# Fireflies-17/Speech-Inpainting

Measured on AMD Instinct MI355X. Metric: real-time factor (audio-sec/wall-sec) per GPU, 4 s clips @16 kHz, 200 ms mask, higher is better.
Workload: dtype encoder GEMMs and attention products: bf16 MFMA, fp32 accumulate (softmax, LayerNorm, head, arg-max in fp32); vocoder: fp16 MFMA (operands rounded to fp16, saturating), fp32 accumulate, activations stored as fp16; 1 GPU; BASELINE configs[1]: batch=32 x 4 s clips per GPU, 200 ms mask, HuBERT-base + HiFi-GAN V1; step = masked log-mel front-end -> encoder -> arg-max/splice -> vocoder on resident raw clips; global_batch=32, clip_samples=64000, mask_frames=10, parallelism=utterance-sharded x1

## Files before the change

speech_inpainting_amd/csrc/api.hip:

```cpp
#include <cmath>
#include <cstdarg>
#include <cstdio>
#include <cstdlib>
#include <cstring>
#include <map>
#include <sstream>
#include <string>
#include <vector>

#include "common.h"

namespace {

struct HostTensor {
    const float* data = nullptr;
    std::vector<long> shape;
    long numel() const { long n = 1; for (long d : shape) n *= d; return n; }
};

struct GemmW {
    size_t w = 0, w_lo = 0, bias = 0;
    int Cin = 0, N = 0, Npad = 0, ntaps = 0, groups = 1, math = 0;
    bool has_bias = false;
};

struct LayerW { GemmW qkv, out, ffn1, ffn2; size_t ln1_g, ln1_b, ln2_g, ln2_b; };
struct ConvW { GemmW g; size_t ln_g = 0, ln_b = 0; };
struct ResW { GemmW c1[SI_MAX_DIL], c2[SI_MAX_DIL]; };

struct Layout {
    size_t total = 0;
    size_t conv0_w, conv0_bias, conv0_g, conv0_b;
    std::vector<ConvW> convs;
    size_t fp_ln_g, fp_ln_b; GemmW proj;
    GemmW pos; size_t enc_ln_g, enc_ln_b;
    std::vector<LayerW> layers;
    size_t head_ln_g, head_ln_b; GemmW head;
    size_t cb_centered, cb_raw, cb_rnorm;
    GemmW pre; std::vector<GemmW> ups; std::vector<ResW> rbs;
    size_t post_w, post_b; int post_C = 0;
    int mel_ld = 0;
};

}

struct si_ctx {
    int device = 0;
    si_model_desc d{};
    char err[512] = {0};
    Layout lay;
    char* wdev = nullptr;
    bool weights_ready = false;
    bool weights_verified = false;
    std::map<std::string, long> dbg_size;
    std::map<std::string, std::pair<float*, long>> dbg_capture;
    struct ProfRec { int name; hipEvent_t a, b; double flops, bytes; };
    bool prof_on = false;
    std::string prof_filter;
    std::vector<std::string> prof_names;
    std::vector<ProfRec> prof_recs;
    std::vector<hipEvent_t> prof_pool;
    size_t prof_used = 0;
    int prof_open = -1;
    int num_cus = 0;
    std::map<const void*, size_t> dyn_lds;
    bool opt_voc_opready = true, opt_voc_res16 = true, opt_enc_opready = true, opt_att_bf16 = true, opt_enc_lingemm = true;
    bool opt_enc_posconv = true;
    int opt_ln_fuse = 1;
    int opt_voc_upsgemm = 1;
    int opt_ffn_pad = 64;
    int opt_gemmcu = 1;
    int opt_voc_chain = 1;
    int opt_voc_fuse = 1;
    char* fe_dev = nullptr;
    size_t fe_dft = 0, fe_hann = 0, fe_basis = 0, fe_lo = 0, fe_hi = 0;
    std::vector<int32_t> vl_host;
    static constexpr int VL_SLOTS = 4;
    int32_t* vl_pin[VL_SLOTS] = {nullptr, nullptr, nullptr, nullptr};
    size_t vl_pin_ints[VL_SLOTS] = {0, 0, 0, 0};
    hipEvent_t vl_ev[VL_SLOTS] = {nullptr, nullptr, nullptr, nullptr};
    int vl_next = 0;
    float* km_cnorm = nullptr;
    int km_cnorm_cap = 0;
};

static char g_create_err[512] = "";

int si_fail(si_ctx* ctx, int code, const char* fmt, ...) {
    char* dst = ctx ? ctx->err : g_create_err;
    va_list ap;
    va_start(ap, fmt);
    vsnprintf(dst, 512, fmt, ap);
    va_end(ap);
    return code;
}
int si_fail_hip(si_ctx* ctx, hipError_t e, const char* what, const char* file, int line) {
    return si_fail(ctx, SI_EHIP, "HIP error %d (%s) at %s:%d: %s", (int)e, hipGetErrorString(e), file, line, what);
}

struct TapSrc { const void* p; long n; int esize = 4; long cols = 0, ld = 0; };
static int si_tap(si_ctx* ctx, hipStream_t st, TapSrc s, const char* fmt, int a = 0, int b = 0, int c = 0) {
    if (ctx->dbg_capture.empty() && strchr(fmt, '%')) return SI_OK;
    char name[48];
    snprintf(name, sizeof(name), fmt, a, b, c);
    ctx->dbg_size[name] = s.n;
    auto it = ctx->dbg_capture.find(name);
    if (it == ctx->dbg_capture.end()) return SI_OK;
    const long m = s.n < it->second.second ? s.n : it->second.second;
    if (m <= 0) return SI_OK;
    if (s.ld > s.cols && s.cols > 0) {
        if (m / s.cols > 0)
            SI_HIP_CHECK(hipMemcpy2DAsync(it->second.first, (size_t)s.cols * s.esize, s.p, (size_t)s.ld * s.esize, (size_t)s.cols * s.esize,
                                          (size_t)(m / s.cols), hipMemcpyDeviceToDevice, st));
    } else {
        SI_HIP_CHECK(hipMemcpyAsync(it->second.first, s.p, (size_t)m * s.esize, hipMemcpyDeviceToDevice, st));
    }
    return SI_OK;
}

void si_prof_begin(si_ctx* ctx, const char* name, double flops, double bytes, hipStream_t st) {
    if (!ctx->prof_on || ctx->prof_used + 2 > ctx->prof_pool.size()) { ctx->prof_open = -1; return; }
    if (!ctx->prof_filter.empty() && ctx->prof_filter != name) { ctx->prof_open = -1; return; }
    int id = -1;
    for (size_t i = 0; i < ctx->prof_names.size(); ++i) if (ctx->prof_names[i] == name) { id = (int)i; break; }
    if (id < 0) { id = (int)ctx->prof_names.size(); ctx->prof_names.push_back(name); }
    si_ctx::ProfRec r{id, ctx->prof_pool[ctx->prof_used], ctx->prof_pool[ctx->prof_used + 1], flops, bytes};
    ctx->prof_used += 2;
    (void)hipEventRecord(r.a, st);
    ctx->prof_open = (int)ctx->prof_recs.size();
    ctx->prof_recs.push_back(r);
}
const char* si_prof_shape_name(const char* name, long M, int N, int K) {
    static const bool on = getenv("SI_PROF_SHAPES") && atoi(getenv("SI_PROF_SHAPES")) != 0;
    if (!on) return name;
    static thread_local char buf[48];
    snprintf(buf, sizeof(buf), "%s_%ldx%dx%d", name, M, N, K);
    return buf;
}
int si_ensure_dyn_lds(si_ctx* ctx, const void* kern, size_t bytes) {
    if (bytes <= 64 * 1024) return SI_OK;
    size_t& have = ctx->dyn_lds[kern];
    if (bytes > have) {
        SI_HIP_CHECK(hipFuncSetAttribute(kern, hipFuncAttributeMaxDynamicSharedMemorySize, (int)bytes));
        have = bytes;
    }
    return SI_OK;
}
int si_opt_gemmcu(const si_ctx* ctx) { return ctx->opt_gemmcu; }
int si_num_cus(si_ctx* ctx) {
    if (ctx->num_cus <= 0) {
        int n = 0;
        if (hipDeviceGetAttribute(&n, hipDeviceAttributeMultiprocessorCount, ctx->device) != hipSuccess || n <= 0) n = 256;
        ctx->num_cus = n;
    }
    return ctx->num_cus;
}
static int vl_upload(si_ctx* ctx, int32_t* dst, hipStream_t st) {
    const size_t n = ctx->vl_host.size();
    const int slot = ctx->vl_next;
    ctx->vl_next = (slot + 1) % si_ctx::VL_SLOTS;
    if (!ctx->vl_ev[slot]) SI_HIP_CHECK(hipEventCreateWithFlags(&ctx->vl_ev[slot], hipEventDisableTiming));
    else SI_HIP_CHECK(hipEventSynchronize(ctx->vl_ev[slot]));
    if (ctx->vl_pin_ints[slot] < n) {
        if (ctx->vl_pin[slot]) SI_HIP_CHECK(hipHostFree(ctx->vl_pin[slot]));
        ctx->vl_pin[slot] = nullptr; ctx->vl_pin_ints[slot] = 0;
        SI_HIP_CHECK(hipHostMalloc(reinterpret_cast<void**>(&ctx->vl_pin[slot]), std::max<size_t>(n, 4096) * sizeof(int32_t), hipHostMallocDefault));
        ctx->vl_pin_ints[slot] = std::max<size_t>(n, 4096);
    }
    memcpy(ctx->vl_pin[slot], ctx->vl_host.data(), n * sizeof(int32_t));
    SI_HIP_CHECK(hipMemcpyAsync(dst, ctx->vl_pin[slot], n * sizeof(int32_t), hipMemcpyHostToDevice, st));
    SI_HIP_CHECK(hipEventRecord(ctx->vl_ev[slot], st));
    return SI_OK;
}
void si_prof_end(si_ctx* ctx, hipStream_t st) {
    if (ctx->prof_open < 0) return;
    (void)hipEventRecord(ctx->prof_recs[ctx->prof_open].b, st);
    ctx->prof_open = -1;
}

namespace {

size_t elem_bytes(int math) { return math == SI_MATH_F32 ? 4 : 2; }

struct Planner {
    size_t cur = 0;
    size_t take(size_t bytes) { size_t o = cur; cur += (bytes + 255) / 256 * 256; return o; }
    size_t floats(size_t n) { return take(n * 4); }
    GemmW gemm(int math, int groups, int ntaps, int N, int Cin, bool bias) {
        GemmW g;
        g.math = math; g.groups = groups; g.ntaps = ntaps; g.N = N; g.Cin = Cin; g.has_bias = bias;
        g.Npad = si_round_up(N, si_pick_bn(N));
        const size_t n = (size_t)groups * ntaps * g.Npad * Cin;
        g.w = take(n * elem_bytes(math));
        if (math == SI_MATH_BF16X3) g.w_lo = take(n * 2);
        if (bias) g.bias = floats((size_t)groups * N);
        return g;
    }
};

int stage_channels(const si_ctx* ctx, int i) {
    const int real = ctx->d.up_initial_channel >> (i + 1);
    const bool r16 = ctx->opt_voc_opready && ctx->opt_voc_res16 && ctx->d.vocoder_math == SI_MATH_F16;
    return (r16 && real < 32 && real >= 4) ? 32 : real;
}

int plan_layout(si_ctx* ctx) {
    const si_model_desc& d = ctx->d;
    Layout& L = ctx->lay;
    Planner P;
    P.take(256);
    const int em = d.encoder_math, vm = d.vocoder_math;
    const int H = d.hidden_size;
    L.conv0_w = P.floats((size_t)d.conv_dim[0] * d.conv_kernel[0]);
    L.conv0_bias = d.conv_bias ? P.floats(d.conv_dim[0]) : 0;
    L.conv0_g = P.floats(d.conv_dim[0]);
    L.conv0_b = P.floats(d.conv_dim[0]);
    L.convs.clear();
    for (int i = 1; i < d.num_conv; ++i) {
        ConvW c;
        c.g = P.gemm(em, 1, d.conv_kernel[i], d.conv_dim[i], d.conv_dim[i - 1], d.conv_bias != 0);
        if (d.feat_norm_layer) { c.ln_g = P.floats(d.conv_dim[i]); c.ln_b = P.floats(d.conv_dim[i]); }
        L.convs.push_back(c);
    }
    const int CF = d.conv_dim[d.num_conv - 1];
    L.fp_ln_g = P.floats(CF); L.fp_ln_b = P.floats(CF);
    L.proj = P.gemm(em, 1, 1, H, CF, true);
    L.pos = P.gemm(em, d.pos_conv_groups, d.pos_conv_kernel, H / d.pos_conv_groups, H / d.pos_conv_groups, true);
    L.enc_ln_g = P.floats(H); L.enc_ln_b = P.floats(H);
    L.layers.clear();
    for (int l = 0; l < d.num_layers; ++l) {
        LayerW w;
// ... 346 lines not shown
    size_t f = 2 * (size_t)B * cmax + BT * d.conv_dim[d.num_conv - 1] + BT * d.hidden_size * 3 + BT * 3 * d.hidden_size + BT * d.intermediate_size +
               (size_t)B * d.conv_dim[0] * 2 + BT * 2;
    const size_t h16 = (BT * d.conv_dim[d.num_conv - 1] + 2 * BT * d.hidden_size + BT * (d.intermediate_size + 128)) * 2;
    return f * 4 + h16 + (size_t)B * 16 + (size_t)B * 4 + si_conv0_partials_bytes(B, N) + 41 * 256 +
           align_up((size_t)(SI_MAX_CONV + 3) * (B + 1) * 4, 256);
}

int vocoder_chunk(const si_model_desc& d, int B) { int c = d.vocoder_chunk > 0 ? d.vocoder_chunk : 32; return std::min(c, std::max(B, 1)); }

long voc_tout(int Tm, int stretch) { return stretch ? (long)std::floor((double)Tm * (441.0 / 256.0)) : Tm; }

size_t vocoder_ws_bytes(const si_ctx* ctx, int B, int Tm, int stretch) {
    const si_model_desc& d = ctx->d;
    const int Bc = vocoder_chunk(d, B);
    const long Tout = voc_tout(Tm, stretch);
    size_t lc_max = (size_t)Tout * d.up_initial_channel;
    long L = Tout; int c = d.up_initial_channel;
    for (int i = 0; i < d.num_ups; ++i) { L *= d.up_rates[i]; c = stage_channels(ctx, i); lc_max = std::max(lc_max, (size_t)L * c); }
    const size_t f = (size_t)Bc * Tout * ctx->lay.mel_ld + 9 * (size_t)Bc * lc_max;
    return f * 4 + 32 * 256 + align_up((size_t)(2 * SI_MAX_UPS + 3) * B * 4, 256);
}

TapGemmParams gemm_params(const si_ctx* ctx, const GemmW& G) {
    TapGemmParams p{};
    p.w = ctx->wdev + G.w;
    p.w_lo = G.math == SI_MATH_BF16X3 ? ctx->wdev + G.w_lo : nullptr;
    p.bias = G.has_bias ? reinterpret_cast<const float*>(ctx->wdev + G.bias) : nullptr;
    p.Cin = G.Cin; p.N = G.N; p.Npad = G.Npad; p.ntaps = G.ntaps; p.groups = G.groups;
    p.stride = 1; p.dil = 1; p.pad = 0; p.pro_slope = 1.f; p.act = SI_ACT_NONE; p.alpha = 1.f; p.accumulate = 0;
    p.out16_slope = 1.f;
    p.nseg = 1;
    return p;
}

struct UpsGeom { int u, pad; long Lout; int M; };
UpsGeom ups_geom(const si_model_desc& d, int i, long Lin) {
    const int u = d.up_rates[i], pad = (d.up_kernels[i] - u) / 2;
    const long Lout = Lin * u;
    return UpsGeom{u, pad, Lout, (int)((pad + Lout - 1) / u + 1)};
}

struct ResLn { const float* stats = nullptr; const float* gamma = nullptr; const float* beta = nullptr; };
struct LinearIo { const unsigned short* x16 = nullptr; unsigned short* y16 = nullptr; int ld_in = 0, ld_out = 0; ResLn res_ln; };
int linear(si_ctx* ctx, const GemmW& G, const float* x, float* y, long rows, int act, const float* res, hipStream_t st, const LinearIo& io = LinearIo()) {
    TapGemmParams p = gemm_params(ctx, G);
    p.x = io.x16 ? nullptr : x; p.x16 = io.x16; p.out = y; p.out16 = io.y16; p.res = res; p.act = act;
    p.res_stats = io.res_ln.stats; p.res_gamma = io.res_ln.gamma; p.res_beta = io.res_ln.beta;
    p.nseg = 1; p.Lin = (int)rows; p.M = (int)rows; p.ldx = io.ld_in ? io.ld_in : G.Cin; p.x_seg_stride = 0;
    p.ldo = io.ld_out ? io.ld_out : G.N; p.o_seg_stride = 0; p.ooff = 0; p.olimit = rows * p.ldo;
    p.lingemm = ctx->opt_enc_lingemm;
    return si_launch_tapgemm(ctx, G.math, p, st);
}

const float* wf(const si_ctx* ctx, size_t off) { return reinterpret_cast<const float*>(ctx->wdev + off); }

}

static int hubert_run(si_ctx* ctx, const float* wav, const int32_t* mask_start, const int32_t* mask_len, const int32_t* valid_len,
                      int normalize, float norm_eps, const double* pre_add, int output_layer, int B, int N, float* out_feats, float* out_hidden,
                      void* workspace, size_t workspace_bytes, si_stream_t stream, const int32_t* host_len = nullptr);

extern "C" {

int si_version(void) { return SI_ABI_VERSION; }

const char* si_last_error(const si_ctx* ctx) { return ctx ? ctx->err : g_create_err; }

int si_create(si_ctx** out, int device_id, const si_model_desc* desc) {
    if (!out) return si_fail(nullptr, SI_EINVAL, "si_create: out is NULL");
    *out = nullptr;
    int rc = check_desc(nullptr, desc);
    if (rc) return rc;
    int ndev = 0;
    if (hipGetDeviceCount(&ndev) != hipSuccess || device_id < 0 || device_id >= ndev)
        return si_fail(nullptr, SI_EHIP, "si_create: device %d not available (%d HIP devices visible)", device_id, ndev);
    si_ctx* ctx = new si_ctx();
    ctx->device = device_id;
    ctx->d = *desc;
    auto env_flag = [](const char* name) { const char* v = getenv(name); return v ? atoi(v) != 0 : true; };
    ctx->opt_voc_opready = env_flag("SI_VOC_OPREADY");
    ctx->opt_voc_res16 = env_flag("SI_VOC_RES16");
    ctx->opt_voc_fuse = getenv("SI_VOC_FUSE") ? atoi(getenv("SI_VOC_FUSE")) : 1;
    ctx->opt_voc_chain = getenv("SI_VOC_CHAIN") ? atoi(getenv("SI_VOC_CHAIN")) : 1;
    ctx->opt_enc_opready = env_flag("SI_ENC_OPREADY");
    ctx->opt_att_bf16 = env_flag("SI_ATT_BF16");
    ctx->opt_enc_lingemm = env_flag("SI_ENC_LINGEMM");
    ctx->opt_enc_posconv = env_flag("SI_ENC_POSCONV");
    ctx->opt_gemmcu = getenv("SI_ENC_GEMMCU") ? atoi(getenv("SI_ENC_GEMMCU")) : 1;
    ctx->opt_ln_fuse = getenv("SI_ENC_LNFUSE") ? atoi(getenv("SI_ENC_LNFUSE")) : 1;
    ctx->opt_voc_upsgemm = getenv("SI_VOC_UPSGEMM") ? atoi(getenv("SI_VOC_UPSGEMM")) : 1;
    ctx->opt_ffn_pad = getenv("SI_ENC_FFNPAD") ? std::min(128, std::max(0, atoi(getenv("SI_ENC_FFNPAD")) / 8 * 8)) : 64;
    plan_layout(ctx);
    *out = ctx;
    return SI_OK;
}

void si_destroy(si_ctx* ctx) {
    if (!ctx) return;
    if (ctx->wdev) { (void)hipSetDevice(ctx->device); (void)hipFree(ctx->wdev); }
    if (ctx->fe_dev) { (void)hipSetDevice(ctx->device); (void)hipFree(ctx->fe_dev); }
    if (ctx->km_cnorm) { (void)hipSetDevice(ctx->device); (void)hipFree(ctx->km_cnorm); }
    for (hipEvent_t e : ctx->prof_pool) (void)hipEventDestroy(e);
    for (int i = 0; i < si_ctx::VL_SLOTS; ++i) {
        if (ctx->vl_ev[i]) { (void)hipEventSynchronize(ctx->vl_ev[i]); (void)hipEventDestroy(ctx->vl_ev[i]); }
        if (ctx->vl_pin[i]) (void)hipHostFree(ctx->vl_pin[i]);
    }
    delete ctx;
}

int si_alloc_weights(si_ctx* ctx) {
    if (!ctx) return SI_EINVAL;
    SI_HIP_CHECK(hipSetDevice(ctx->device));
    if (!ctx->wdev) SI_HIP_CHECK(hipMalloc(reinterpret_cast<void**>(&ctx->wdev), ctx->lay.total));
    ctx->weights_ready = true;
    ctx->weights_verified = false;
    return SI_OK;
}

int si_load_weights(si_ctx* ctx, const void* host_blob, size_t nbytes, const char* index) {
    if (!ctx || !host_blob || !index) return si_fail(ctx, SI_EINVAL, "si_load_weights: NULL argument");
    Packer P;
    P.ctx = ctx;
    int rc = parse_index(ctx, index, host_blob, nbytes, P.t);
    if (rc) return rc;
    rc = pack_weights(ctx, P);
    if (rc) return rc;
    SI_HIP_CHECK(hipSetDevice(ctx->device));
    if (!ctx->wdev) SI_HIP_CHECK(hipMalloc(reinterpret_cast<void**>(&ctx->wdev), ctx->lay.total));
    const BlobHeader hd = blob_header(ctx);
    memcpy(P.out.data(), &hd, sizeof(hd));
    SI_HIP_CHECK(hipMemcpy(ctx->wdev, P.out.data(), ctx->lay.total, hipMemcpyHostToDevice));
    ctx->weights_ready = true;
    ctx->weights_verified = true;
    return SI_OK;
}

int si_weights_check(si_ctx* ctx) {
    if (!ctx) return SI_EINVAL;
    if (!ctx->wdev) return si_fail(ctx, SI_ESTATE, "weights are not allocated: call si_load_weights or si_alloc_weights first");
    SI_HIP_CHECK(hipSetDevice(ctx->device));
    BlobHeader got{};
    SI_HIP_CHECK(hipMemcpy(&got, ctx->wdev, sizeof(got), hipMemcpyDeviceToHost));
    const BlobHeader want = blob_header(ctx);
    if (got.magic != want.magic || got.version != want.version || got.fingerprint != want.fingerprint || got.total != want.total)
        return si_fail(ctx, SI_EWEIGHTS, "the weight blob in this context was packed for a different layout (fingerprint %016llx / %llu bytes, this "
                       "context plans %016llx / %llu): the source rank's model desc or SI_VOC_* environment differs, or the broadcast has not arrived",
                       (unsigned long long)got.fingerprint, (unsigned long long)got.total, (unsigned long long)want.fingerprint, (unsigned long long)want.total);
    ctx->weights_verified = true;
    return SI_OK;
}

int si_weights_device_ptr(si_ctx* ctx, void** ptr, size_t* nbytes) {
    if (!ctx || !ptr || !nbytes) return si_fail(ctx, SI_EINVAL, "si_weights_device_ptr: NULL argument");
    if (!ctx->wdev) return si_fail(ctx, SI_ESTATE, "weights are not allocated: call si_load_weights or si_alloc_weights first");
    *ptr = ctx->wdev;
    *nbytes = ctx->lay.total;
    return SI_OK;
}

int si_num_frames(const si_ctx* ctx, int N) { return ctx ? enc_dims(ctx->d, N).T : SI_EINVAL; }

int si_vocoder_samples(const si_ctx* ctx, int Tm, int stretch) {
    if (!ctx) return SI_EINVAL;
    long L = voc_tout(Tm, stretch);
    for (int i = 0; i < ctx->d.num_ups; ++i) L *= ctx->d.up_rates[i];
    return (int)L;
// ... 989 lines not shown
```

speech_inpainting_amd/csrc/common.h:

```cpp
#pragma once
#include <hip/hip_runtime.h>
#include <stdint.h>

#include "../../include/si_hip.h"

#define SI_HIP_CHECK(expr)                                                                      \
    do {                                                                                        \
        hipError_t _e = (expr);                                                                 \
        if (_e != hipSuccess) return si_fail_hip(ctx, _e, #expr, __FILE__, __LINE__);           \
    } while (0)

int si_fail_hip(si_ctx* ctx, hipError_t e, const char* what, const char* file, int line);
int si_fail(si_ctx* ctx, int code, const char* fmt, ...);
void si_prof_begin(si_ctx* ctx, const char* name, double flops, double bytes, hipStream_t st);
void si_prof_end(si_ctx* ctx, hipStream_t st);
const char* si_prof_shape_name(const char* name, long M, int N, int K);
int si_ensure_dyn_lds(si_ctx* ctx, const void* kern, size_t bytes);
int si_num_cus(si_ctx* ctx);

typedef unsigned short bf16_t;

struct SiVlTile { int b, row0, L; };
#ifdef __HIPCC__
__device__ __forceinline__ SiVlTile si_vl_tile(const int32_t* __restrict__ lens, int B, int step, int t) {
// ... 141 lines not shown
                              const float* cb_rnorm , int K, float* mel, int Tm, int64_t* labels, hipStream_t st,
                              const int32_t* frame_cnt = nullptr );

int si_launch_code_splice(si_ctx* ctx, const int64_t* clean, const int64_t* masked, const int32_t* first, const int32_t* last, int B, int T,
                          int64_t* out, hipStream_t st);

int si_launch_codebook_gather(si_ctx* ctx, const int64_t* labels, int B, int D, const int32_t* frame_pos, int Lm,
                              const float* cb_raw, int K, float* mel, int Tm, hipStream_t st);

int si_launch_kmeans_assign(si_ctx* ctx, const float* x, long rows, int D, const float* cent, int K, int64_t* labels, float* dist,
                            hipStream_t st, float* cnorm_scratch = nullptr);

int si_launch_codebook_metrics(si_ctx* ctx, const float* feats, int B, int T, int D, const int32_t* frame_pos, int Lm,
                               const float* cb_centered, const float* cb_rnorm, int K, const int64_t* target, float* terms,
                               float* loss, int64_t* pred, float* cos_pt, hipStream_t st);

int si_launch_mel_metrics(si_ctx* ctx, const float* a, const float* b, int B, int D, int L, const float* center, float* out, hipStream_t st);
int si_launch_sisdr(si_ctx* ctx, const float* est, const float* ref, int B, int n, float* out, hipStream_t st);

int si_launch_wave_peak(si_ctx* ctx, const float* wav, const int32_t* ms, const int32_t* me, int B, int N, float* peak,
                        hipStream_t st, const int32_t* n_len = nullptr);
int si_launch_mel_frames(si_ctx* ctx, const float* wav, const int32_t* ms, const int32_t* me, const float* peak,
                         const float* hann, int B, int N, int Tm, int hop, int pad, int nfft, int kc, int normalize, float* frames,
                         hipStream_t st, const int32_t* n_len = nullptr, const int32_t* tm_len = nullptr);
int si_launch_mel_project(si_ctx* ctx, const float* spec, int ld_spec, int nbin, int im_off, const float* basis_t, const int32_t* lo,
                          const int32_t* hi, int nmel, int B, int Tm, float* mel, hipStream_t st, const int32_t* tm_len = nullptr);

int si_launch_resample_poly(si_ctx* ctx, const float* x, int B, int n_in, const float* taps, int ntaps, int up, int down,
                            int pre_remove, int n_out, float* y, hipStream_t st);

int si_launch_resample_sinc(si_ctx* ctx, const float* x, const int32_t* n_len, int B, int n_in, const double* win, const double* dwin, int nwin,
                            int num_table, int step, double scale, double ratio, const double* time_reg, int n_out, float* y, hipStream_t st);
int si_launch_pcm16(si_ctx* ctx, const float* wav, long n, int16_t* out, hipStream_t st);

__device__ __forceinline__ float si_gelu_fast(float x) {
    const float z = x * 0.70710678118654752440f;
    const float az = __builtin_fabsf(z);
    const float t = __builtin_amdgcn_rcpf(fmaf(0.3275911f, az, 1.0f));
    float poly = fmaf(1.061405429f, t, -1.453152027f);
    poly = fmaf(poly, t, 1.421413741f);
    poly = fmaf(poly, t, -0.284496736f);
    poly = fmaf(poly, t, 0.254829592f);
    poly *= t;
    const float e = __builtin_amdgcn_exp2f(-az * az * 1.4426950408889634f);
    const float erf = __builtin_copysignf(fmaf(-poly, e, 1.0f), z);
    return 0.5f * x * (1.0f + erf);
}

__device__ __forceinline__ float si_ln_apply(float x, float mean, float rstd, float g, float b) { return fmaf((x - mean) * rstd, g, b); }

__device__ __forceinline__ float si_lrelu01(float v) {
    float r;
    asm("v_max_f32 %0, %1, %2" : "=v"(r) : "v"(v), "v"(0.1f * v));
    return r;
}

struct UpsampleParams {
    const unsigned short* x16;
    const unsigned short* w;
    const float* bias;
    unsigned short* out16;
    int B, Lin, M;
    int Cin, N, taps;
    long ooff;
    long o_clip_stride, o_clip_elems;
    const int32_t* lens_lin; const int32_t* lens_m; const int32_t* lens_m_host;
    int total_tiles;
};
int si_launch_upsample_stream(si_ctx* ctx, const UpsampleParams& p, hipStream_t st);

struct ResPairParams {
    const unsigned short* y16;
    unsigned short* out16;
    const unsigned short* w1;
    const unsigned short* w2;
    const float* b1;
    const float* b2;
    int B, L, k, dil;
    float alpha;
    int accumulate;
    const int32_t* lens; const int32_t* lens_host;
    int total_tiles;
    float out_slope;
};
int si_launch_respair_wide(si_ctx* ctx, int C, const ResPairParams& p, hipStream_t st);
struct ResChainParams {
    const unsigned short* y16;
    unsigned short* out16;
    const unsigned short* w1[3];
    const unsigned short* w2[3];
    const float* b1[3];
    const float* b2[3];
    int B, L, k;
    int dil[3];
    float alpha;
    int accumulate;
    const int32_t* lens; const int32_t* lens_host;
    int total_tiles;
};
int si_launch_reschain(si_ctx* ctx, int C, const ResChainParams& p, hipStream_t st);
int si_launch_respair(si_ctx* ctx, int C, const unsigned short* y16, unsigned short* out16, const void* w1, const void* w2,
                      const float* b1, const float* b2, int B, int L, int k, int dil, float alpha, int accumulate, hipStream_t st,
                      const int32_t* lens = nullptr, const int32_t* lens_host = nullptr, float out_slope = 1.f);

int si_launch_extend_mel(si_ctx* ctx, const float* mel, int B, int D, int Tm, int Tout, int stretch, float* out, int ldo,
                         hipStream_t st, const int32_t* tm_len = nullptr, const int32_t* tout_len = nullptr);
int si_launch_extend_mel_cf(si_ctx* ctx, const float* mel, int B, int D, int Tm, int Tout, float* out, hipStream_t st);
int si_launch_small_conv1d(si_ctx* ctx, const float* x, const float* w, const float* bias, const float* res, float* y, int B, int Cin,
                           int Tin, int Cout, int Tout, int K, int stride, int dil, int pad, int relu_in, int channels_last, hipStream_t st);
int si_launch_f0enc_fused(si_ctx* ctx, const float* weights, const float* f0, int B, int T, float* h_out, int in_width, int out_width, int width,
                          int n_state, int depth, int down_t, int stride_t, int growth, int dk, int dpad, double macs, hipStream_t st);
int si_launch_unit_frontend(si_ctx* ctx, const int64_t* code, int Fc, const int64_t* f0_code, int Fp, const float* spk_emb,
                            const float* emb_c, int Kc, const float* emb_p, int Kp, int E, int B, float* out, hipStream_t st);
int si_launch_conv_post(si_ctx* ctx, const float* x, const float* w , const float* bias, int B, int L, int C, int k,
                        float* wav, hipStream_t st, const unsigned short* x16 = nullptr ,
                        const int32_t* lens = nullptr, const int32_t* lens_host = nullptr);
```

speech_inpainting_amd/csrc/respair_wide.hip:

```cpp
#include <algorithm>
#include <cstdio>
#include <cstdlib>

#include "common.h"

typedef float f32x4 __attribute__((ext_vector_type(4)));
typedef unsigned int u32x4 __attribute__((ext_vector_type(4)));
typedef unsigned int u32x2 __attribute__((ext_vector_type(2)));
typedef _Float16 f16x8 __attribute__((ext_vector_type(8)));
typedef _Float16 f16x4 __attribute__((ext_vector_type(4)));

template <int ROWB>
__device__ __forceinline__ int swz16(int row) {
    if constexpr (ROWB >= 256) return (row & 7) << 5;
    else return ((row >> 1) & 3) << 5;
}

#ifdef RPW_TIMELINE
__device__ unsigned long long rpw_tl[2][10];
#define RPW_TL_DECL unsigned long long tl_t = wall_clock64(); unsigned long long tl_acc[6] = {0, 0, 0, 0, 0, 0}; unsigned long long tl_tiles = 0; unsigned long long tl_w = 0, tl_sub[2] = {0, 0};
#define RPW_TL_W0 tl_w = wall_clock64();
#define RPW_TL_W1(q) tl_sub[q] += wall_clock64() - tl_w;
#define RPW_TL(ph) { const unsigned long long n_ = wall_clock64(); tl_acc[ph] += n_ - tl_t; tl_t = n_; }
#define RPW_TL_TILE ++tl_tiles;
#define RPW_TL_FLUSH if (threadIdx.x == 0) { for (int q_ = 0; q_ < 6; ++q_) atomicAdd(&rpw_tl[C == 256][q_], tl_acc[q_]); atomicAdd(&rpw_tl[C == 256][6], tl_tiles); atomicAdd(&rpw_tl[C == 256][7], 1ull); atomicAdd(&rpw_tl[C == 256][8], tl_sub[0]); atomicAdd(&rpw_tl[C == 256][9], tl_sub[1]); }
extern "C" int si_debug_rpw_timeline(unsigned long long* out, int reset) {
    if (hipMemcpyFromSymbol(out, HIP_SYMBOL(rpw_tl), sizeof(rpw_tl)) != hipSuccess) return -1;
    if (reset) { unsigned long long z[2][10] = {}; if (hipMemcpyToSymbol(HIP_SYMBOL(rpw_tl), z, sizeof(z)) != hipSuccess) return -1; }
    return 0;
}
#else
#define RPW_TL_DECL
#define RPW_TL_W0
#define RPW_TL_W1(q)
#define RPW_TL(ph)
#define RPW_TL_TILE
#define RPW_TL_FLUSH
#endif

constexpr int RPW_HALO = 50;

template <int C, int R1, int WARPS_M, int WARPS_N, int BKW, bool ACC, bool VL>
__global__ __launch_bounds__(64 * WARPS_M * WARPS_N, 2) void respair_wide_kernel(const ResPairParams p) {
    static_assert((WARPS_M * WARPS_N == 8 || WARPS_M * WARPS_N == 4) && R1 == WARPS_M * 64 && C == WARPS_N * 64, "64 x 64 wave tiles");
    static_assert(BKW == 128 || BKW == 64, "weight-slab depth");
    constexpr int NT = 64 * WARPS_M * WARPS_N;
    constexpr int ROWBY = C * 2;
    constexpr int ROWBW = BKW * 2;
    constexpr int ROWBO = C * 4;
    constexpr int CPRY = C / 8, CPRW = BKW / 8;
    constexpr int NCH = C / BKW;
    constexpr int KS = BKW / 32;
    constexpr int YBYTES = (R1 + RPW_HALO) * ROWBY;
    constexpr int WBYTES = C * ROWBW;
    constexpr int WSLOTS = C * CPRW / NT;
    constexpr int YSLOTS = ((R1 + RPW_HALO) * CPRY + NT - 1) / NT;
    constexpr int YRPP = NT / CPRY, WRPP = NT / CPRW;
    static_assert(C * CPRW % NT == 0 && NT % CPRY == 0 && NT % CPRW == 0, "staging maps");
    static_assert(R1 * ROWBO <= YBYTES + 2 * WBYTES, "the output image reuses the operand region (not the biases behind it)");

    __builtin_amdgcn_s_setreg((0 << 11) | (23 << 6) | 1, 1);
    extern __shared__ __attribute__((aligned(16))) char smem[];
    char* const Ys = smem;
    char* const Ws = smem + YBYTES;
    float* const Bs = reinterpret_cast<float*>(smem + YBYTES + 2 * WBYTES);

    const int tid = threadIdx.x, lane = tid & 63, wave = tid >> 6;
    const int r16 = lane & 15, kg = lane >> 4;
    const int wm0 = (wave / WARPS_N) * 64, wn0 = (wave % WARPS_N) * 64;
    const int k = p.k, d = p.dil;
    const int p1 = d * (k - 1) / 2, p2 = (k - 1) / 2;
    const int BMo = R1 - (k - 1);
    const int R0 = R1 + (k - 1) * d;
    const int tiles_x = (p.L + BMo - 1) / BMo;
    const int total = VL ? p.total_tiles : tiles_x * p.B;
    auto tile_of = [&](int t, int& tb, int& tm0, int& tL) {
        if constexpr (VL) { const SiVlTile v = si_vl_tile(p.lens, p.B, BMo, t); tb = v.b; tm0 = v.row0; tL = v.L; }
        else { tb = t / tiles_x; tm0 = (t - tb * tiles_x) * BMo; tL = p.L; }
    };
    const __amdgpu_buffer_rsrc_t w1rsrc = __builtin_amdgcn_make_buffer_rsrc(const_cast<unsigned short*>(p.w1), 0, k * C * C * 2, 0x00020000);
    const __amdgpu_buffer_rsrc_t w2rsrc = __builtin_amdgcn_make_buffer_rsrc(const_cast<unsigned short*>(p.w2), 0, k * C * C * 2, 0x00020000);

    const int NS1 = k * NCH, NS = 2 * NS1;
    const int wc = tid % CPRW, wr0 = tid / CPRW;
    u32x4 rw[WSLOTS];
    auto issueW1 = [&](int s, int i) {
        const bool second = s >= NS1;
        const int q = second ? s - NS1 : s;
        const int tap = q / NCH, ch = q - tap * NCH;
        const int soff = __builtin_amdgcn_readfirstlane((tap * C * C + ch * BKW) * 2);
        const int n = wr0 + i * WRPP;
        rw[i] = __builtin_amdgcn_raw_buffer_load_b128(second ? w2rsrc : w1rsrc, (n * C + 8 * wc) * 2, soff, 0);
    };
    auto issueW = [&](int s) {
#pragma unroll
        for (int i = 0; i < WSLOTS; ++i) issueW1(s, i);
    };
    auto storeW1 = [&](char* dst, int i) {
        const int n = wr0 + i * WRPP;
        *reinterpret_cast<u32x4*>(dst + n * ROWBW + ((wc << 4) ^ swz16<ROWBW>(n))) = rw[i];
    };
    auto storeW = [&](char* dst) {
#pragma unroll
        for (int i = 0; i < WSLOTS; ++i) storeW1(dst, i);
    };
    const int yc = tid % CPRY, yr0 = tid / CPRY;
    u32x4 ry[YSLOTS];
    auto issueY = [&](int t) {
        int tb, tm0, tL;
        tile_of(t, tb, tm0, tL);
        const int trow0 = tm0 - p2 - p1;
        const __amdgpu_buffer_rsrc_t rs = __builtin_amdgcn_make_buffer_rsrc(const_cast<unsigned short*>(p.y16 + (long)tb * p.L * C), 0, tL * C * 2, 0x00020000);
#pragma unroll
        for (int i = 0; i < YSLOTS; ++i)
            ry[i] = __builtin_amdgcn_raw_buffer_load_b128(rs, ((trow0 + yr0 + i * YRPP) * C + 8 * yc) * 2, 0, 0);
    };

    if (tid < C / 2) {
        const int which = tid / (C / 4), c4 = (tid % (C / 4)) * 4;
        *reinterpret_cast<f32x4*>(Bs + which * C + c4) = *reinterpret_cast<const f32x4*>((which ? p.b2 : p.b1) + c4);
    }
    const int preW = (wn0 + r16) * ROWBW + (swz16<ROWBW>(wn0 + r16) ^ (kg << 4));
    issueW(0);
    issueY(blockIdx.x);
    RPW_TL_DECL

  for (int tile = blockIdx.x; tile < total; tile += gridDim.x) {
    const int nxt = tile + (int)gridDim.x < total ? tile + (int)gridDim.x : tile;
    int b, m0, Lb;
    tile_of(tile, b, m0, Lb);
    const int t_row0 = m0 - p2;
    const long seg = (long)b * p.L * C;
    const __amdgpu_buffer_rsrc_t yrsrc = __builtin_amdgcn_make_buffer_rsrc(const_cast<unsigned short*>(p.y16 + seg), 0, Lb * C * 2, 0x00020000);
    const __amdgpu_buffer_rsrc_t orsrc = __builtin_amdgcn_make_buffer_rsrc(p.out16 + seg, 0, Lb * C * 2, 0x00020000);

    storeW(Ws);
    issueW(1);
#pragma unroll
    for (int i = 0; i < YSLOTS; ++i) {
        const int r = yr0 + i * YRPP;
        if ((i + 1) * YRPP <= R1 || r < R0) {
            f16x8 h = __builtin_bit_cast(f16x8, ry[i]);
            h = __builtin_elementwise_max(h, h * (_Float16)0.1f);
            *reinterpret_cast<f16x8*>(Ys + r * ROWBY + ((yc << 4) ^ swz16<ROWBY>(r))) = h;
        }
    }
    __syncthreads();
    RPW_TL(0)

    f32x4 acc[4][4];
    auto init_acc = [&](const float* bias) {
#pragma unroll
        for (int j = 0; j < 4; ++j) {
            const f32x4 bv = *reinterpret_cast<const f32x4*>(bias + wn0 + 16 * j + 4 * kg);
#pragma unroll
            for (int i = 0; i < 4; ++i) acc[i][j] = bv;
        }
    };
    init_acc(Bs);
    auto compute = [&](int roff, int cb16, const char* Wc, auto&& hook) {
        const int r0 = wm0 + r16 + roff;
        const int preY = r0 * ROWBY + (swz16<ROWBY>(r0) ^ (kg << 4));
        auto load = [&](f16x8 (&y)[4], f16x8 (&w)[4], int ks) {
            const char* yp = Ys + (preY ^ (cb16 + ks * 64));
            const char* wp = Wc + (preW ^ (ks * 64));
#pragma unroll
            for (int i = 0; i < 4; ++i) y[i] = *reinterpret_cast<const f16x8*>(yp + i * (16 * ROWBY));
#pragma unroll
            for (int j = 0; j < 4; ++j) w[j] = *reinterpret_cast<const f16x8*>(wp + j * (16 * ROWBW));
        };
        auto mma = [&](const f16x8 (&y)[4], const f16x8 (&w)[4]) {
#pragma unroll
            for (int i = 0; i < 4; ++i)
#pragma unroll
                for (int j = 0; j < 4; ++j) acc[i][j] = __builtin_amdgcn_mfma_f32_16x16x32_f16(w[j], y[i], acc[i][j], 0, 0, 0);
        };
        f16x8 ya[4], wa[4], yb[4], wb[4];
        load(ya, wa, 0);
#pragma unroll
        for (int ks = 0; ks < KS; ks += 2) {
            load(yb, wb, ks + 1);
            __builtin_amdgcn_sched_barrier(0);
            __builtin_amdgcn_s_setprio(1);
            mma(ya, wa);
            __builtin_amdgcn_s_setprio(0);
            __builtin_amdgcn_sched_barrier(0);
            hook(ks);
            if (ks + 2 < KS) load(ya, wa, ks + 2);
            __builtin_amdgcn_sched_barrier(0);
            __builtin_amdgcn_s_setprio(1);
            mma(yb, wb);
            __builtin_amdgcn_s_setprio(0);
            __builtin_amdgcn_sched_barrier(0);
            hook(ks + 1);
        }
    };

    int tap = 0, ch = 0;
    for (int s = 0; s < NS - 1; ++s) {
        const bool second = s >= NS1;
        char* const Wn = Ws + ((s + 1) & 1) * WBYTES;
        static_assert(WSLOTS % KS == 0, "the slab's stores are spread evenly over its k-steps");
        compute(second ? tap : tap * d, ch * (BKW * 2), Ws + (s & 1) * WBYTES, [&](int ks) {
            const int s2 = s + 2 < NS ? s + 2 : NS - 1;
#pragma unroll
            for (int i = 0; i < WSLOTS / KS; ++i) {
                storeW1(Wn, ks * (WSLOTS / KS) + i);
                issueW1(s2, ks * (WSLOTS / KS) + i);
            }
        });
        if (s == NS1 - 1) {
            __syncthreads();
            RPW_TL(1)
#pragma unroll
            for (int ip = 0; ip < 2; ++ip) {
                float inside[2];
#pragma unroll
                for (int u = 0; u < 2; ++u) {
                    const int grow = t_row0 + wm0 + 16 * (2 * ip + u) + r16;
                    inside[u] = (grow >= 0 && grow < Lb) ? 1.f : 0.f;
                }
                const int ms = wm0 + 16 * (2 * ip + (kg & 1)) + r16;
#pragma unroll
                for (int j = 0; j < 4; ++j) {
                    u32x2 pk[2];
#pragma unroll
                    for (int u = 0; u < 2; ++u) {
                        f16x4 hv;
#pragma unroll
                        for (int e = 0; e < 4; ++e) hv[e] = (_Float16)(si_lrelu01(acc[2 * ip + u][j][e]) * inside[u]);
                        pk[u] = __builtin_bit_cast(u32x2, hv);
                    }
#pragma unroll
                    for (int q = 0; q < 2; ++q) {
                        const auto r = __builtin_amdgcn_permlane16_swap(pk[0][q], pk[1][q], false, false);
                        pk[0][q] = r[0]; pk[1][q] = r[1];
                    }
                    const int ch = ((wn0 + 16 * j) >> 3) + (kg >> 1);
                    *reinterpret_cast<u32x4*>(Ys + ms * ROWBY + ((ch << 4) ^ swz16<ROWBY>(ms))) = u32x4{pk[0][0], pk[0][1], pk[1][0], pk[1][1]};
                }
            }
            init_acc(Bs + C);
            RPW_TL(2)
        }
        if (++ch == NCH) { ch = 0; if (++tap == k) tap = 0; }
        __syncthreads();
    }
    if constexpr (!ACC) issueY(nxt);
    __builtin_amdgcn_sched_barrier(0);
    compute(tap, ch * (BKW * 2), Ws + ((NS - 1) & 1) * WBYTES, [](int) {});
    RPW_TL(3)
    constexpr int ORPP = NT / CPRY;
    constexpr int OPASS = R1 / ORPP;
    const int c8 = tid % CPRY, or0 = tid / CPRY;
    u32x4 res[OPASS], prev[ACC ? OPASS : 1];
    int goff[OPASS];
#pragma unroll
    for (int it = 0; it < OPASS; ++it) {
        const int o = or0 + it * ORPP;
        const int grow = m0 + o;
        goff[it] = (o < BMo && grow < Lb) ? (grow * C + 8 * c8) * 2 : (int)0x80000000;
        res[it] = __builtin_amdgcn_raw_buffer_load_b128(yrsrc, goff[it], 0, 0);
        if constexpr (ACC) prev[it] = __builtin_amdgcn_raw_buffer_load_b128(orsrc, goff[it], 0, 0);
    }
    RPW_TL_W0
    __syncthreads();
    RPW_TL_W1(0)
    RPW_TL_W0

#pragma unroll
    for (int i = 0; i < 4; ++i) {
        const int m = wm0 + 16 * i + r16;
#pragma unroll
        for (int j = 0; j < 4; ++j) {
            const int co = ((wn0 + 16 * j) >> 2) + kg;
            *reinterpret_cast<f32x4*>(smem + m * ROWBO + ((co ^ (m & 15)) << 4)) = acc[i][j];
        }
    }
    RPW_TL_W1(1)
    __syncthreads();
    RPW_TL(4)
    issueW(0);
    {
        const bool oact = p.out_slope != 0.f && p.out_slope != 1.f;
#pragma unroll
        for (int it = 0; it < OPASS; ++it) {
            const int o = or0 + it * ORPP;
            const f32x4 a0 = *reinterpret_cast<const f32x4*>(smem + o * ROWBO + (((2 * c8) ^ (o & 15)) << 4));
            const f32x4 a1 = *reinterpret_cast<const f32x4*>(smem + o * ROWBO + (((2 * c8 + 1) ^ (o & 15)) << 4));
            const f16x8 rh = __builtin_bit_cast(f16x8, res[it]);
            f16x8 ph = {};
            if constexpr (ACC) ph = __builtin_bit_cast(f16x8, prev[it]);
            f16x8 out;
#pragma unroll
            for (int e = 0; e < 8; ++e) {
                const float a = e < 4 ? a0[e] : a1[e - 4];
                float v = (a + (float)rh[e]) * p.alpha;
                if constexpr (ACC) v += (float)ph[e];
                if (oact) v = v > 0.f ? v : v * p.out_slope;
                out[e] = (_Float16)v;
            }
            __builtin_amdgcn_raw_buffer_store_b128(__builtin_bit_cast(u32x4, out), orsrc, goff[it], 0, 0);
        }
    }
    if constexpr (ACC) issueY(nxt);
    __syncthreads();
    RPW_TL(5)
    RPW_TL_TILE
  }
  RPW_TL_FLUSH
}

template <int C, int R1, int WARPS_M, int WARPS_N, int BKW>
static int respair_wide_launch(si_ctx* ctx, const ResPairParams& p0, hipStream_t st) {
    const ResPairParams& p = p0;
    const int BMo = R1 - (p.k - 1);
    const size_t lds = (size_t)(R1 + RPW_HALO) * C * 2 + 2 * (size_t)C * BKW * 2 + 2 * (size_t)C * 4;
    const bool vl = p0.lens != nullptr;
    auto kern = vl ? (p.accumulate ? respair_wide_kernel<C, R1, WARPS_M, WARPS_N, BKW, true, true> : respair_wide_kernel<C, R1, WARPS_M, WARPS_N, BKW, false, true>)
                   : (p.accumulate ? respair_wide_kernel<C, R1, WARPS_M, WARPS_N, BKW, true, false> : respair_wide_kernel<C, R1, WARPS_M, WARPS_N, BKW, false, false>);
    if (int rc = si_ensure_dyn_lds(ctx, reinterpret_cast<const void*>(kern), lds)) return rc;
    const int total = vl ? (int)si_vl_tiles(p.lens_host, p.B, BMo) : ((p.L + BMo - 1) / BMo) * p.B;
    if (total <= 0) return SI_OK;
    ResPairParams pk = p0;
    pk.total_tiles = total;
    const int grid = std::min(total, si_num_cus(ctx) * (WARPS_M * WARPS_N == 4 ? 2 : 1));
    char name[48];
    snprintf(name, sizeof(name), p.accumulate ? "respair_f16_c%d_acc" : "respair_f16_c%d", C);
    double rows = (double)p.B * p.L;
    if (vl) { rows = 0; for (int b = 0; b < p.B; ++b) rows += p.lens_host[b]; }
    const double elems = rows * C;
    si_prof_begin(ctx, name, 2.0 * 2.0 * elems * C * p.k, elems * (2.0 + 2.0 + (p.accumulate ? 2.0 : 0.0)) + 2.0 * 2.0 * p.k * C * C, st);
    hipLaunchKernelGGL(kern, dim3(grid), dim3(64 * WARPS_M * WARPS_N), lds, st, pk);
    si_prof_end(ctx, st);
    SI_HIP_CHECK(hipGetLastError());
    return SI_OK;
}

int si_launch_respair_wide(si_ctx* ctx, int C, const ResPairParams& p, hipStream_t st) {
    if (C == 128) return respair_wide_launch<128, 256, 4, 2, 128>(ctx, p, st);
    if (C == 256) return respair_wide_launch<256, 128, 2, 4, 64>(ctx, p, st);
    return 1;
}
```

Measured before the change: 11350 x real-time (audio-sec/wall-sec); `value` = whole-job aggregate over n_gpus, `value_per_gpu` = the per-GPU figure the metric names.

## Carry conv1 halo rows across consecutive tiles in C=128 residual-pair kernel

For the C=128 residual-pair vocoder kernel, each workgroup now walks a segment of several consecutive row tiles. It keeps the last k-1 rows of the intermediate conv1 output in an LDS side buffer (a porch), so the next tile can write full R1 output rows instead of R1-(k-1). This removes the recomputation of overlapping halo rows between adjacent tiles. The host picks the segment length by simulating per-workgroup load balance, which trades fewer, longer segments (worse balance) against less redundant work. It also adds LDS for the porch and side buffer.

```diff
diff --git a/speech_inpainting_amd/csrc/api.hip b/speech_inpainting_amd/csrc/api.hip
--- a/speech_inpainting_amd/csrc/api.hip
+++ b/speech_inpainting_amd/csrc/api.hip
@@ -71,6 +71,7 @@
     int opt_ffn_pad = 64;
     int opt_gemmcu = 1;
     int opt_voc_chain = 1;
+    int opt_voc_carry = 1;
     int opt_voc_fuse = 1;
     char* fe_dev = nullptr;
     size_t fe_dft = 0, fe_hann = 0, fe_basis = 0, fe_lo = 0, fe_hi = 0;
@@ -147,6 +148,7 @@
     return SI_OK;
 }
 int si_opt_gemmcu(const si_ctx* ctx) { return ctx->opt_gemmcu; }
+int si_opt_voc_carry(const si_ctx* ctx) { return ctx->opt_voc_carry; }
 int si_num_cus(si_ctx* ctx) {
     if (ctx->num_cus <= 0) {
         int n = 0;
@@ -659,6 +661,7 @@
     ctx->opt_voc_res16 = env_flag("SI_VOC_RES16");
     ctx->opt_voc_fuse = getenv("SI_VOC_FUSE") ? atoi(getenv("SI_VOC_FUSE")) : 1;
     ctx->opt_voc_chain = getenv("SI_VOC_CHAIN") ? atoi(getenv("SI_VOC_CHAIN")) : 1;
+    ctx->opt_voc_carry = getenv("SI_VOC_CARRY") ? std::max(0, atoi(getenv("SI_VOC_CARRY"))) : 1;
     ctx->opt_enc_opready = env_flag("SI_ENC_OPREADY");
     ctx->opt_att_bf16 = env_flag("SI_ATT_BF16");
     ctx->opt_enc_lingemm = env_flag("SI_ENC_LINGEMM");
diff --git a/speech_inpainting_amd/csrc/common.h b/speech_inpainting_amd/csrc/common.h
--- a/speech_inpainting_amd/csrc/common.h
+++ b/speech_inpainting_amd/csrc/common.h
@@ -247,7 +247,9 @@
     const int32_t* lens; const int32_t* lens_host;
     int total_tiles;
     float out_slope;
-};
+    int carry_n;
+};
+int si_opt_voc_carry(const si_ctx* ctx);
 int si_launch_respair_wide(si_ctx* ctx, int C, const ResPairParams& p, hipStream_t st);
 struct ResChainParams {
     const unsigned short* y16;
diff --git a/speech_inpainting_amd/csrc/respair_wide.hip b/speech_inpainting_amd/csrc/respair_wide.hip
--- a/speech_inpainting_amd/csrc/respair_wide.hip
+++ b/speech_inpainting_amd/csrc/respair_wide.hip
@@ -39,6 +39,7 @@
 #endif
 
 constexpr int RPW_HALO = 50;
+constexpr int RPW_PORCH = 16;
 
 template <int C, int R1, int WARPS_M, int WARPS_N, int BKW, bool ACC, bool VL>
 __global__ __launch_bounds__(64 * WARPS_M * WARPS_N, 2) void respair_wide_kernel(const ResPairParams p) {
@@ -58,12 +59,18 @@
     constexpr int YRPP = NT / CPRY, WRPP = NT / CPRW;
     static_assert(C * CPRW % NT == 0 && NT % CPRY == 0 && NT % CPRW == 0, "staging maps");
     static_assert(R1 * ROWBO <= YBYTES + 2 * WBYTES, "the output image reuses the operand region (not the biases behind it)");
+    constexpr bool CARRY = C == 128;
+    constexpr int PORCH = CARRY ? RPW_PORCH : 0;
+    constexpr int PBYTES = PORCH * ROWBY;
+    static_assert(RPW_PORCH == 16 && R1 >= RPW_PORCH && PBYTES <= NT * 16, "porch");
 
     __builtin_amdgcn_s_setreg((0 << 11) | (23 << 6) | 1, 1);
     extern __shared__ __attribute__((aligned(16))) char smem[];
     char* const Ys = smem;
-    char* const Ws = smem + YBYTES;
-    float* const Bs = reinterpret_cast<float*>(smem + YBYTES + 2 * WBYTES);
+    char* const Img = smem + PBYTES;
+    char* const Ws = Img + YBYTES;
+    float* const Bs = reinterpret_cast<float*>(Img + YBYTES + 2 * WBYTES);
+    char* const Side = Img + YBYTES + 2 * WBYTES + 2 * C * 4;
 
     const int tid = threadIdx.x, lane = tid & 63, wave = tid >> 6;
     const int r16 = lane & 15, kg = lane >> 4;
@@ -72,11 +79,15 @@
     const int p1 = d * (k - 1) / 2, p2 = (k - 1) / 2;
     const int BMo = R1 - (k - 1);
     const int R0 = R1 + (k - 1) * d;
-    const int tiles_x = (p.L + BMo - 1) / BMo;
+    const int seg_n = CARRY ? p.carry_n : 1;
+    const int seg_rows = BMo + (seg_n - 1) * R1;
+    const int tiles_x = (p.L + seg_rows - 1) / seg_rows;
     const int total = VL ? p.total_tiles : tiles_x * p.B;
-    auto tile_of = [&](int t, int& tb, int& tm0, int& tL) {
-        if constexpr (VL) { const SiVlTile v = si_vl_tile(p.lens, p.B, BMo, t); tb = v.b; tm0 = v.row0; tL = v.L; }
-        else { tb = t / tiles_x; tm0 = (t - tb * tiles_x) * BMo; tL = p.L; }
+    auto tile_of = [&](int sg, int j, int& tb, int& tt0, int& tL) {
+        int row0;
+        if constexpr (VL) { const SiVlTile v = si_vl_tile(p.lens, p.B, seg_rows, sg); tb = v.b; row0 = v.row0; tL = v.L; }
+        else { tb = sg / tiles_x; row0 = (sg - tb * tiles_x) * seg_rows; tL = p.L; }
+        tt0 = row0 - p2 + j * R1;
     };
     const __amdgpu_buffer_rsrc_t w1rsrc = __builtin_amdgcn_make_buffer_rsrc(const_cast<unsigned short*>(p.w1), 0, k * C * C * 2, 0x00020000);
     const __amdgpu_buffer_rsrc_t w2rsrc = __builtin_amdgcn_make_buffer_rsrc(const_cast<unsigned short*>(p.w2), 0, k * C * C * 2, 0x00020000);
@@ -106,10 +117,10 @@
     };
     const int yc = tid % CPRY, yr0 = tid / CPRY;
     u32x4 ry[YSLOTS];
-    auto issueY = [&](int t) {
-        int tb, tm0, tL;
-        tile_of(t, tb, tm0, tL);
-        const int trow0 = tm0 - p2 - p1;
+    auto issueY = [&](int sg, int j) {
+        int tb, tt0, tL;
+        tile_of(sg, j, tb, tt0, tL);
+        const int trow0 = tt0 - p1;
         const __amdgpu_buffer_rsrc_t rs = __builtin_amdgcn_make_buffer_rsrc(const_cast<unsigned short*>(p.y16 + (long)tb * p.L * C), 0, tL * C * 2, 0x00020000);
 #pragma unroll
         for (int i = 0; i < YSLOTS; ++i)
@@ -122,14 +133,19 @@
     }
     const int preW = (wn0 + r16) * ROWBW + (swz16<ROWBW>(wn0 + r16) ^ (kg << 4));
     issueW(0);
-    issueY(blockIdx.x);
+    issueY(blockIdx.x, 0);
     RPW_TL_DECL
 
-  for (int tile = blockIdx.x; tile < total; tile += gridDim.x) {
-    const int nxt = tile + (int)gridDim.x < total ? tile + (int)gridDim.x : tile;
-    int b, m0, Lb;
-    tile_of(tile, b, m0, Lb);
-    const int t_row0 = m0 - p2;
+  for (int sg = blockIdx.x, tj = 0; sg < total;) {
+    int b, t_row0, Lb;
+    tile_of(sg, tj, b, t_row0, Lb);
+    const bool carried = CARRY && tj > 0;
+    int nsg = sg, nj = tj;
+    if (CARRY && tj + 1 < seg_n && t_row0 + R1 - p2 < Lb) nj = tj + 1;
+    else if (sg + (int)gridDim.x < total) { nsg = sg + (int)gridDim.x; nj = 0; }
+    const int m0 = carried ? t_row0 - p2 : t_row0 + p2;
+    const int keep = carried ? R1 : BMo;
+    const int c2off = carried ? PORCH - (k - 1) : PORCH;
     const long seg = (long)b * p.L * C;
     const __amdgpu_buffer_rsrc_t yrsrc = __builtin_amdgcn_make_buffer_rsrc(const_cast<unsigned short*>(p.y16 + seg), 0, Lb * C * 2, 0x00020000);
     const __amdgpu_buffer_rsrc_t orsrc = __builtin_amdgcn_make_buffer_rsrc(p.out16 + seg, 0, Lb * C * 2, 0x00020000);
@@ -142,8 +158,11 @@
         if ((i + 1) * YRPP <= R1 || r < R0) {
             f16x8 h = __builtin_bit_cast(f16x8, ry[i]);
             h = __builtin_elementwise_max(h, h * (_Float16)0.1f);
-            *reinterpret_cast<f16x8*>(Ys + r * ROWBY + ((yc << 4) ^ swz16<ROWBY>(r))) = h;
-        }
+            *reinterpret_cast<f16x8*>(Ys + (r + PORCH) * ROWBY + ((yc << 4) ^ swz16<ROWBY>(r))) = h;
+        }
+    }
+    if constexpr (CARRY) {
+        if (carried && tid < PBYTES / 16) *reinterpret_cast<u32x4*>(Ys + tid * 16) = *reinterpret_cast<const u32x4*>(Side + tid * 16);
     }
     __syncthreads();
     RPW_TL(0)
@@ -201,7 +220,7 @@
         const bool second = s >= NS1;
         char* const Wn = Ws + ((s + 1) & 1) * WBYTES;
         static_assert(WSLOTS % KS == 0, "the slab's stores are spread evenly over its k-steps");
-        compute(second ? tap : tap * d, ch * (BKW * 2), Ws + (s & 1) * WBYTES, [&](int ks) {
+        compute(second ? tap + c2off : tap * d + PORCH, ch * (BKW * 2), Ws + (s & 1) * WBYTES, [&](int ks) {
             const int s2 = s + 2 < NS ? s + 2 : NS - 1;
 #pragma unroll
             for (int i = 0; i < WSLOTS / KS; ++i) {
@@ -237,7 +256,12 @@
                         pk[0][q] = r[0]; pk[1][q] = r[1];
                     }
                     const int ch = ((wn0 + 16 * j) >> 3) + (kg >> 1);
-                    *reinterpret_cast<u32x4*>(Ys + ms * ROWBY + ((ch << 4) ^ swz16<ROWBY>(ms))) = u32x4{pk[0][0], pk[0][1], pk[1][0], pk[1][1]};
+                    const u32x4 tv = u32x4{pk[0][0], pk[0][1], pk[1][0], pk[1][1]};
+                    *reinterpret_cast<u32x4*>(Ys + (ms + PORCH) * ROWBY + ((ch << 4) ^ swz16<ROWBY>(ms))) = tv;
+                    if constexpr (CARRY) {
+                        if (ip == 1 && wm0 == R1 - 64 && (kg & 1))
+                            *reinterpret_cast<u32x4*>(Side + (ms - (R1 - PORCH)) * ROWBY + ((ch << 4) ^ swz16<ROWBY>(ms))) = tv;
+                    }
                 }
             }
             init_acc(Bs + C);
@@ -246,9 +270,9 @@
         if (++ch == NCH) { ch = 0; if (++tap == k) tap = 0; }
         __syncthreads();
     }
-    if constexpr (!ACC) issueY(nxt);
+    if constexpr (!ACC) issueY(nsg, nj);
     __builtin_amdgcn_sched_barrier(0);
-    compute(tap, ch * (BKW * 2), Ws + ((NS - 1) & 1) * WBYTES, [](int) {});
+    compute(tap + c2off, ch * (BKW * 2), Ws + ((NS - 1) & 1) * WBYTES, [](int) {});
     RPW_TL(3)
     constexpr int ORPP = NT / CPRY;
     constexpr int OPASS = R1 / ORPP;
@@ -259,7 +283,7 @@
     for (int it = 0; it < OPASS; ++it) {
         const int o = or0 + it * ORPP;
         const int grow = m0 + o;
-        goff[it] = (o < BMo && grow < Lb) ? (grow * C + 8 * c8) * 2 : (int)0x80000000;
+        goff[it] = (o < keep && grow < Lb) ? (grow * C + 8 * c8) * 2 : (int)0x80000000;
         res[it] = __builtin_amdgcn_raw_buffer_load_b128(yrsrc, goff[it], 0, 0);
         if constexpr (ACC) prev[it] = __builtin_amdgcn_raw_buffer_load_b128(orsrc, goff[it], 0, 0);
     }
@@ -274,7 +298,7 @@
 #pragma unroll
         for (int j = 0; j < 4; ++j) {
             const int co = ((wn0 + 16 * j) >> 2) + kg;
-            *reinterpret_cast<f32x4*>(smem + m * ROWBO + ((co ^ (m & 15)) << 4)) = acc[i][j];
+            *reinterpret_cast<f32x4*>(Img + m * ROWBO + ((co ^ (m & 15)) << 4)) = acc[i][j];
         }
     }
     RPW_TL_W1(1)
@@ -286,8 +310,8 @@
 #pragma unroll
         for (int it = 0; it < OPASS; ++it) {
             const int o = or0 + it * ORPP;
-            const f32x4 a0 = *reinterpret_cast<const f32x4*>(smem + o * ROWBO + (((2 * c8) ^ (o & 15)) << 4));
-            const f32x4 a1 = *reinterpret_cast<const f32x4*>(smem + o * ROWBO + (((2 * c8 + 1) ^ (o & 15)) << 4));
+            const f32x4 a0 = *reinterpret_cast<const f32x4*>(Img + o * ROWBO + (((2 * c8) ^ (o & 15)) << 4));
+            const f32x4 a1 = *reinterpret_cast<const f32x4*>(Img + o * ROWBO + (((2 * c8 + 1) ^ (o & 15)) << 4));
             const f16x8 rh = __builtin_bit_cast(f16x8, res[it]);
             f16x8 ph = {};
             if constexpr (ACC) ph = __builtin_bit_cast(f16x8, prev[it]);
@@ -303,28 +327,78 @@
             __builtin_amdgcn_raw_buffer_store_b128(__builtin_bit_cast(u32x4, out), orsrc, goff[it], 0, 0);
         }
     }
-    if constexpr (ACC) issueY(nxt);
+    if constexpr (ACC) issueY(nsg, nj);
     __syncthreads();
     RPW_TL(5)
     RPW_TL_TILE
+    if constexpr (CARRY) { if (nsg == sg && nj == tj) break; sg = nsg; tj = nj; }
+    else sg += (int)gridDim.x;
   }
   RPW_TL_FLUSH
+}
+
+struct RpwWalk { long segments; int most; };
+static RpwWalk rpw_walk(const int32_t* lens, int B, int L, int k, int cus, int n, int R1) {
+    const int step = n * R1 - (k - 1);
+    long segs = 0;
+    for (int b = 0; b < B; ++b) { const int Lb = lens ? lens[b] : L; if (Lb > 0) segs += (Lb + step - 1) / step; }
+    const int grid = (int)std::min<long>(segs, cus);
+    if (grid <= 0) return RpwWalk{0, 0};
+    int load[1024];
+    std::fill(load, load + grid, 0);
+    int g = 0;
+    for (int b = 0; b < B; ++b) {
+        const int Lb = lens ? lens[b] : L;
+        for (int row0 = 0; row0 < Lb; row0 += step) {
+            const int left = Lb - row0;
+            load[g] += left >= step ? n : (left + (k - 1) + R1 - 1) / R1;
+            if (++g == grid) g = 0;
+        }
+    }
+    return RpwWalk{segs, *std::max_element(load, load + grid)};
+}
+static int rpw_plan(const int32_t* lens, int B, int L, int k, int cus, int carry, int R1, int* most) {
+    int Lmax = 0;
+    for (int b = 0; b < B; ++b) Lmax = std::max(Lmax, lens ? lens[b] : L);
+    const int nmax = std::max(1, (Lmax + R1 - 1) / R1);
+    cus = std::min(std::max(cus, 1), 1024);
+    int best_n = carry >= 2 ? std::min(carry, nmax) : 1;
+    int best = rpw_walk(lens, B, L, k, cus, best_n, R1).most;
+    if (carry == 1) {
+        long fewest = 0;
+        for (int b = 0; b < B; ++b) { const int Lb = lens ? lens[b] : L; if (Lb > 0) fewest += (Lb + (k - 1) + R1 - 1) / R1; }
+        const long bound = (fewest + cus - 1) / cus;
+        for (int n = 2; n <= nmax && best > bound; ++n) {
+            const int m = rpw_walk(lens, B, L, k, cus, n, R1).most;
+            if (m < best) { best = m; best_n = n; }
+        }
+    }
+    if (most) *most = best;
+    return best_n;
+}
+extern "C" int si_debug_rpw_plan(const int32_t* lens, int B, int L, int k, int cus, int carry, int* most) {
+    if (B <= 0 || k < 3 || k > 11 || (k & 1) == 0 || (!lens && L <= 0)) return -1;
+    return rpw_plan(lens, B, L, k, cus, carry, 256, most);
 }
 
 template <int C, int R1, int WARPS_M, int WARPS_N, int BKW>
 static int respair_wide_launch(si_ctx* ctx, const ResPairParams& p0, hipStream_t st) {
     const ResPairParams& p = p0;
-    const int BMo = R1 - (p.k - 1);
-    const size_t lds = (size_t)(R1 + RPW_HALO) * C * 2 + 2 * (size_t)C * BKW * 2 + 2 * (size_t)C * 4;
+    constexpr bool CARRY = C == 128;
+    const size_t lds = (size_t)(R1 + RPW_HALO + (CARRY ? 2 * RPW_PORCH : 0)) * C * 2 + 2 * (size_t)C * BKW * 2 + 2 * (size_t)C * 4;
     const bool vl = p0.lens != nullptr;
     auto kern = vl ? (p.accumulate ? respair_wide_kernel<C, R1, WARPS_M, WARPS_N, BKW, true, true> : respair_wide_kernel<C, R1, WARPS_M, WARPS_N, BKW, false, true>)
                    : (p.accumulate ? respair_wide_kernel<C, R1, WARPS_M, WARPS_N, BKW, true, false> : respair_wide_kernel<C, R1, WARPS_M, WARPS_N, BKW, false, false>);
     if (int rc = si_ensure_dyn_lds(ctx, reinterpret_cast<const void*>(kern), lds)) return rc;
-    const int total = vl ? (int)si_vl_tiles(p.lens_host, p.B, BMo) : ((p.L + BMo - 1) / BMo) * p.B;
+    const int wgs = si_num_cus(ctx) * (WARPS_M * WARPS_N == 4 ? 2 : 1);
+    ResPairParams pk = p0;
+    pk.carry_n = 1;
+    if (CARRY) pk.carry_n = p0.carry_n > 0 ? p0.carry_n : rpw_plan(p.lens_host, p.B, p.L, p.k, wgs, si_opt_voc_carry(ctx), R1, nullptr);
+    const int seg_rows = pk.carry_n * R1 - (p.k - 1);
+    const int total = vl ? (int)si_vl_tiles(p.lens_host, p.B, seg_rows) : ((p.L + seg_rows - 1) / seg_rows) * p.B;
     if (total <= 0) return SI_OK;
-    ResPairParams pk = p0;
     pk.total_tiles = total;
-    const int grid = std::min(total, si_num_cus(ctx) * (WARPS_M * WARPS_N == 4 ? 2 : 1));
+    const int grid = std::min(total, wgs);
     char name[48];
     snprintf(name, sizeof(name), p.accumulate ? "respair_f16_c%d_acc" : "respair_f16_c%d", C);
     double rows = (double)p.B * p.L;
```

Result: no change. 11350 x real-time (audio-sec/wall-sec); `value` = whole-job aggregate over n_gpus, `value_per_gpu` = the per-GPU figure the metric names (-0.0%).
